# omid-arhami/topolow

Measured on AMD Instinct MI355X. Metric: relaxation iterations/sec (NxN pairs), higher is better.
Workload: dtype f32

## Files before the change

topolow_amd/csrc/relax_kernels.h:

```cpp
#pragma once

#include <hip/hip_runtime.h>
#include <type_traits>
#include "relax_common.h"
#include "relax_prep_types.h"

namespace topolow {

constexpr int kThreads = 256;
constexpr int kWaves = kThreads / 64;

template <int THREADS_, int RPW_, int CHUNK_, int PRIO_ = 0, int MINWAVES_ = 1>
struct StageCfg {
  static constexpr int MINWAVES = MINWAVES_;
  static constexpr int PRIO = PRIO_;
  static constexpr int THREADS = THREADS_;
  static constexpr int WAVES = THREADS_ / 64;
  static constexpr int RPW = RPW_;
  static constexpr int ROWS = WAVES * RPW_;
  static constexpr int CHUNK = CHUNK_;
};

template <typename real> struct Math;
template <> struct Math<float> {
// ... 760 lines not shown
    part_cnt[blockIdx.x] = tc;
  }
}

__global__ __launch_bounds__(1024) void reduce_push_kernel(
    const double* __restrict__ part_sum, const unsigned long long* __restrict__ part_cnt, int n_parts,
    double* const* __restrict__ dst_sum, unsigned long long* const* __restrict__ dst_cnt, int n_dst,
    int slot, const RunState* st) {
  if (st != nullptr && st->stopped) return;
  __shared__ double sh_s[1024];
  __shared__ unsigned long long sh_c[1024];
  double s = 0.0;
  unsigned long long c = 0;
  for (int p = threadIdx.x; p < n_parts; p += 1024) { s += part_sum[p]; c += part_cnt[p]; }
  sh_s[threadIdx.x] = s;
  sh_c[threadIdx.x] = c;
  __syncthreads();
  for (int half = 512; half >= 1; half >>= 1) {
    if (threadIdx.x < half) {
      sh_s[threadIdx.x] += sh_s[threadIdx.x + half];
      sh_c[threadIdx.x] += sh_c[threadIdx.x + half];
    }
    __syncthreads();
  }
  if ((int)threadIdx.x < n_dst) {
    dst_sum[threadIdx.x][slot] = sh_s[0];
    dst_cnt[threadIdx.x][slot] = sh_c[0];
  }
}

__global__ __launch_bounds__(1024) void reduce_total_kernel(
    const double* __restrict__ part_sum, const unsigned long long* __restrict__ part_cnt, int n_parts,
    double* __restrict__ out2, const RunState* st) {
  if (st != nullptr && st->stopped) { if (threadIdx.x == 0) { out2[0] = 0.0; out2[1] = 0.0; } return; }
  __shared__ double sh_s[1024];
  __shared__ unsigned long long sh_c[1024];
  double s = 0.0;
  unsigned long long c = 0;
  for (int p = threadIdx.x; p < n_parts; p += 1024) { s += part_sum[p]; c += part_cnt[p]; }
  sh_s[threadIdx.x] = s;
  sh_c[threadIdx.x] = c;
  __syncthreads();
  for (int half = 512; half >= 1; half >>= 1) {
    if (threadIdx.x < half) {
      sh_s[threadIdx.x] += sh_s[threadIdx.x + half];
      sh_c[threadIdx.x] += sh_c[threadIdx.x + half];
    }
    __syncthreads();
  }
  if (threadIdx.x == 0) { out2[0] = sh_s[0]; out2[1] = (double)sh_c[0]; }
}

constexpr int kCtlThreads = 1024;

template <int THREADS, typename real>
__device__ __forceinline__ void controller_step(
    RunState* st, RunState* mailbox, const double* __restrict__ part_sum,
    const unsigned long long* __restrict__ part_cnt, int n_parts, const real* __restrict__ pos,
    real* __restrict__ best_pos, long long n_values, int iter1, double k_after,
    double* __restrict__ trace, int trace_cap, const double* __restrict__ total2) {
  static_assert(THREADS >= 64 && THREADS <= kCtlThreads && kCtlThreads % THREADS == 0 && (THREADS & (THREADS - 1)) == 0,
                "controller_step: a power-of-two workgroup of at most kCtlThreads threads");
  constexpr int V = kCtlThreads / THREADS;
  if (st->stopped) return;
  __shared__ double sh_s[THREADS];
  __shared__ unsigned long long sh_c[THREADS];
  __shared__ int sh_action;
  double s[V];
  unsigned long long c[V];
#pragma unroll
  for (int j = 0; j < V; ++j) {
    s[j] = 0.0;
    c[j] = 0;
    if (total2 == nullptr)
      for (int p = threadIdx.x + j * THREADS; p < n_parts; p += kCtlThreads) { s[j] += part_sum[p]; c[j] += part_cnt[p]; }
  }
  if (total2 != nullptr && threadIdx.x == 0) { s[0] = total2[0]; c[0] = (unsigned long long)total2[1]; }
#pragma unroll
  for (int h = V / 2; h >= 1; h >>= 1) {
#pragma unroll
    for (int j = 0; j < h; ++j) { s[j] += s[j + h]; c[j] += c[j + h]; }
  }
  sh_s[threadIdx.x] = s[0];
  sh_c[threadIdx.x] = c[0];
  __syncthreads();
  for (int half = THREADS / 2; half >= 1; half >>= 1) {
    if (threadIdx.x < half) {
      sh_s[threadIdx.x] += sh_s[threadIdx.x + half];
      sh_c[threadIdx.x] += sh_c[threadIdx.x + half];
    }
    __syncthreads();
  }
  if (threadIdx.x == 0) {
    const double err = sh_c[0] > 0 ? sh_s[0] / (double)sh_c[0] : 0.0;
    const int action = st->ctl.observe(err, iter1, k_after);
    st->last_mae = err;
    if (trace != nullptr && st->n_checks < trace_cap) {
      trace[3 * st->n_checks + 0] = (double)iter1;
      trace[3 * st->n_checks + 1] = err;
      trace[3 * st->n_checks + 2] = k_after;
    }
    st->n_checks += 1;
    st->iter_base = iter1;
    st->k_base = k_after;
    if (action & 1) { st->stopped = 1; st->converged = 1; }
    sh_action = action;
  }
  __syncthreads();
  if (sh_action & 2) {
    const long long bytes = n_values * (long long)sizeof(real);
    const long long n16 = bytes / 16;
    const uint4* src = reinterpret_cast<const uint4*>(pos);
    uint4* dst = reinterpret_cast<uint4*>(best_pos);
    for (long long q = threadIdx.x; q < n16; q += THREADS) dst[q] = src[q];
    for (long long q = n16 * 16 / (long long)sizeof(real) + threadIdx.x; q < n_values; q += THREADS)
      best_pos[q] = pos[q];
  }
  __syncthreads();
  if (threadIdx.x == 0 && mailbox != nullptr) {
    *mailbox = *st;
    __threadfence_system();
  }
}

template <typename real>
__global__ __launch_bounds__(kCtlThreads) void controller_kernel(
    RunState* st, RunState* mailbox, const double* __restrict__ part_sum,
    const unsigned long long* __restrict__ part_cnt, int n_parts, const real* __restrict__ pos,
    real* __restrict__ best_pos, long long n_values, int iter1, double k_after,
    double* __restrict__ trace, int trace_cap, const double* __restrict__ total2) {
  controller_step<kCtlThreads, real>(st, mailbox, part_sum, part_cnt, n_parts, pos, best_pos, n_values, iter1, k_after,
                                     trace, trace_cap, total2);
}

__global__ __launch_bounds__(kThreads) void encode_dense_kernel(
    const double* __restrict__ D, const int* __restrict__ T, int n, int row_begin, int row_end,
    int ld, uint32_t* __restrict__ out, const int* __restrict__ perm, float* __restrict__ dout) {
  const int c = blockIdx.y * kThreads + threadIdx.x;
  const int i = row_begin + blockIdx.x;
  if (c >= ld || i >= row_end) return;
  uint32_t w = kInfWord;
  float dl = 0.0f;
  if (c < n && c != i) {
    const int oi = perm ? perm[i] : i, oc = perm ? perm[c] : c;
    const int lo = oi < oc ? oi : oc, hi = oi < oc ? oc : oi;
    const size_t cell = (size_t)lo + (size_t)hi * n;
    w = encode_target(D[cell], T[cell]);
    dl = encode_delta(D[cell], w);
  }
  out[enc_index(i - row_begin, c, ld)] = w;
  if (dout != nullptr) dout[enc_index(i - row_begin, c, ld)] = dl;
}


__global__ __launch_bounds__(kPrepThreads) void prep_degree_terms_kernel(const int32_t* __restrict__ degrees, int n,
                                                                          const int* __restrict__ perm,
                                                                          float* __restrict__ gplus) {
  const int q = blockIdx.x * kPrepThreads + threadIdx.x;
  if (q >= n) return;
  gplus[q] = (float)degrees[perm != nullptr ? perm[q] : q] + 1.0f;
}

__global__ __launch_bounds__(kPrepThreads) void prep_session_edges_kernel(
    const int32_t* __restrict__ edge_i, const int32_t* __restrict__ edge_j, const double* __restrict__ edge_dist,
    const int32_t* __restrict__ edge_thresh, long long n_edges, const int* __restrict__ inv, int* __restrict__ ei,
    int* __restrict__ ej, int8_t* __restrict__ ec, double* __restrict__ t64, float* __restrict__ t32) {
  const long long e = (long long)blockIdx.x * kPrepThreads + threadIdx.x;
  if (e >= n_edges) return;
  const int a = edge_i[e], b = edge_j[e];
  ei[e] = inv != nullptr ? inv[a] : a;
  ej[e] = inv != nullptr ? inv[b] : b;
  const int c = edge_thresh[e];
  ec[e] = (int8_t)(c == 0 ? 0 : (c == 1 ? 1 : (c == -1 ? -1 : 2)));
  const double d = edge_dist[e];
  if (t64 != nullptr) t64[e] = d;
  else t32[e] = (float)d;
}

TL_HD inline uint64_t cell_fingerprint(int lo, int hi, uint32_t word) {
  return mix64(((uint64_t)(uint32_t)lo << 32) ^ (uint64_t)(uint32_t)hi ^ ((uint64_t)word * 0x9e3779b97f4a7c15ull));
}
TL_HD inline bool dense_takes(int i, int c, bool parity) {
  if (!parity) return c > i;
  const bool even = ((i + c) & 1) == 0;
  return (even & (c > i)) | (!even & (c < i));
// ... 77 lines not shown
```

topolow_amd/csrc/relax_symm.h:

```cpp
#pragma once

#include <hip/hip_runtime.h>
#include <algorithm>
#include <type_traits>
#include <vector>
#include "relax_common.h"
#include "relax_kernels.h"
#include "relax_symm_plan.h"

namespace topolow {

#ifndef TOPOLOW_SYM_MINW
#define TOPOLOW_SYM_MINW 2
#endif

typedef float symf2 __attribute__((ext_vector_type(2)));
#ifdef TOPOLOW_SYM_STAMPS
__device__ unsigned long long* g_sym_stamps = nullptr;
#endif

#define TL_SYM_DPP_ADD(v, ctrl) asm volatile("v_add_f32_dpp %0, %0, %0 " ctrl " row_mask:0xf bank_mask:0xf" : "+v"(v))
template <int NV>
__device__ __forceinline__ void sym_col_reduce(float (&first)[NV], float (&second)[NV]) {
#pragma unroll
// ... 269 lines not shown
    if constexpr (ERR) {
      double s = (double)err_unit;
#pragma unroll
      for (int m = 32; m >= 1; m >>= 1) s += __shfl_xor(s, m, 64);
      if constexpr (ANYTHR) {
#pragma unroll
        for (int m = 32; m >= 1; m >>= 1) cnt_unit2 += __shfl_xor(cnt_unit2, m, 64);
      }
      if (lane == 0) {
        part_sum[slot] = s;
        part_cnt[slot] = ANYTHR ? (unsigned long long)cnt_unit2 : (slot == 0 ? fixed_cnt : 0ull);
      }
    }
  }
#ifdef TOPOLOW_SYM_STAMPS
  if (lane == 0 && g_sym_stamps != nullptr) {
    g_sym_stamps[4 * gw] = __builtin_amdgcn_s_memtime() - stamp_c0;
    g_sym_stamps[4 * gw + 1] = stamp_r0;
    g_sym_stamps[4 * gw + 2] = __builtin_amdgcn_s_memrealtime();
    unsigned hw_id, xcc_id;
    asm volatile("s_getreg_b32 %0, hwreg(HW_REG_HW_ID)" : "=s"(hw_id));
    asm volatile("s_getreg_b32 %0, hwreg(HW_REG_XCC_ID)" : "=s"(xcc_id));
    g_sym_stamps[4 * gw + 3] = ((unsigned long long)xcc_id << 32) | hw_id;
  }
#endif
}

template <int DIM, typename real> struct SymReal;
template <int DIM> struct SymReal<DIM, float> {
  static constexpr int W = SymRec<DIM>::W;
  __device__ static float ks(double k, float g) { return (float)(2.0 * k) / (4.0f * g + (float)k); }
  __device__ static float cg(double c_rep, float g) { return (float)(0.5 * c_rep) / g; }
  __device__ static float far(int) { return kFarF32; }
};

struct SymApplyCheck {
  const double* part_sum = nullptr;
  const unsigned long long* part_cnt = nullptr;
  int n_parts = 0;
  const void* pos = nullptr;
  void* best = nullptr;
  long long n_values = 0;
  int iter1 = 0;
  double k_after = 0.0;
  double* trace = nullptr;
  int trace_cap = 0;
  RunState* mailbox = nullptr;
};

#ifndef TL_APPLY_PARTS
#define TL_APPLY_PARTS 16
#endif
constexpr int kSymApplyParts = TL_APPLY_PARTS;
template <int DIM, typename real>
__global__ __launch_bounds__(32 * kSymApplyParts) void symm_apply_kernel(
    const real* __restrict__ rec, real* __restrict__ rec_next, real* __restrict__ pos_out, const float* __restrict__ gplus,
    const real* __restrict__ rowpart, const real* __restrict__ colpart, const int2* __restrict__ row_units, int n,
    int npad, double k_next, double c_rep, int iter1, RunState* st, int rr_stages = 0, int rr_stage = 0,
    SymApplyCheck chk = SymApplyCheck{}) {
  const bool check_wg = (int)blockIdx.x * kSymCols >= npad;
  const int R = check_wg ? 0 : blockIdx.x >> 1;
  const int2 ru = row_units[R];
  int stopped = st->stopped;
  asm("" : "+s"(stopped) : "s"(ru.x), "s"(ru.y), "s"(rec), "s"(rowpart), "s"(colpart), "s"(n), "s"(npad), "s"(rr_stages), "s"(rr_stage),
      "s"(rec_next), "s"(pos_out), "s"(gplus), "s"(k_next), "s"(c_rep));
  if (stopped) return;
  if (check_wg) {
    if (chk.part_sum != nullptr)
      controller_step<32 * kSymApplyParts, real>(st, chk.mailbox, chk.part_sum, chk.part_cnt, chk.n_parts,
                                                 (const real*)chk.pos, (real*)chk.best, chk.n_values, chk.iter1,
                                                 chk.k_after, chk.trace, chk.trace_cap, nullptr);
    return;
  }
  using T = SymReal<DIM, real>;
  constexpr int W = T::W;
  constexpr int kWavesA = kSymApplyParts / 2;
  __shared__ real red[kWavesA][kSymCols][DIM];
  const int part = threadIdx.x >> 5, pt = threadIdx.x & 31;
  const int i = blockIdx.x * kSymCols + pt;
  real acc[DIM];
#pragma unroll
  for (int d = 0; d < DIM; ++d) acc[d] = 0;
  int rp0 = 0, rp1 = R;
  if (rr_stages > 0) sym_rr_above(npad / kSymRows, rr_stages, rr_stage, R, rp0, rp1);
  for (int Rp = rp0 + part; Rp < rp1; Rp += kSymApplyParts) {
    const real* src = colpart + ((size_t)Rp * npad + i) * DIM;
#pragma unroll
    for (int d = 0; d < DIM; ++d) acc[d] += src[d];
  }
  const int row_in_tile = i - R * kSymRows;
  for (int q = part; q < ru.y; q += kSymApplyParts) {
    const real* src = rowpart + ((size_t)(ru.x + q) * kSymRows + row_in_tile) * DIM;
#pragma unroll
    for (int d = 0; d < DIM; ++d) acc[d] -= src[d];
  }
#pragma unroll
  for (int d = 0; d < DIM; ++d) {
    if constexpr (std::is_same<real, float>::value) acc[d] += __shfl_xor(acc[d], 32, 64);
    else acc[d] += T::lane_xor(acc[d], 32);
  }
  const int wave = threadIdx.x >> 6;
  if ((threadIdx.x & 32) == 0) {
#pragma unroll
    for (int d = 0; d < DIM; ++d) red[wave][pt][d] = acc[d];
  }
  __syncthreads();
  if (part == 0 && i < n) {
    bool finite = true;
    real out[DIM];
#pragma unroll
    for (int d = 0; d < DIM; ++d) {
      real t = red[0][pt][d];
#pragma unroll
      for (int p = 1; p < kWavesA; ++p) t += red[p][pt][d];
      out[d] = rec[(size_t)i * W + d] + t;
      finite = finite && isfinite(out[d]);
      pos_out[(size_t)i * DIM + d] = out[d];
      rec_next[(size_t)i * W + d] = out[d];
    }
    const real g = (real)gplus[i];
    rec_next[(size_t)i * W + DIM] = T::ks(k_next, g);
    rec_next[(size_t)i * W + DIM + 1] = T::cg(c_rep, g);
    if (!finite) atomicMin(&st->first_nonfinite, iter1);
  }
}

template <int DIM, typename real>
__global__ __launch_bounds__(256) void symm_records_kernel(const real* __restrict__ pos, const float* __restrict__ gplus,
                                                          real* __restrict__ rec, int n, int npad, double k, double c_rep) {
  using T = SymReal<DIM, real>;
  constexpr int W = T::W;
  const int i = blockIdx.x * blockDim.x + threadIdx.x;
  if (i >= npad) return;
  real* r = rec + (size_t)i * W;
  if (i < n) {
#pragma unroll
    for (int d = 0; d < DIM; ++d) r[d] = pos[(size_t)i * DIM + d];
    const real g = (real)gplus[i];
    r[DIM] = T::ks(k, g);
    r[DIM + 1] = T::cg(c_rep, g);
  } else {
#pragma unroll
    for (int d = 0; d < DIM; ++d) r[d] = T::far(d);
    r[DIM] = 0;
    r[DIM + 1] = 0;
  }
#pragma unroll
// ... 107 lines not shown
```

topolow_amd/csrc/topolow_relax.hip:

```cpp

#include "topolow_session.h"
#include "topolow_prep.h"
#include "relax_kernels.h"
#include "relax_exact.h"
#include "relax_tilegs.h"
#include "relax_symm.h"
#include "relax_symm64.h"
#include "relax_symm_wide.h"
#include "relax_cv.h"

namespace {

#define TL_DISPATCH_DIM(dim, FN, ...)                 \
  switch (dim) {                                      \
    case 1: FN<1>(__VA_ARGS__); break;                \
    case 2: FN<2>(__VA_ARGS__); break;                \
    case 3: FN<3>(__VA_ARGS__); break;                \
    case 4: FN<4>(__VA_ARGS__); break;                \
    case 5: FN<5>(__VA_ARGS__); break;                \
    case 6: FN<6>(__VA_ARGS__); break;                \
    case 7: FN<7>(__VA_ARGS__); break;                \
    case 8: FN<8>(__VA_ARGS__); break;                \
    case 9: FN<9>(__VA_ARGS__); break;                \
    case 10: FN<10>(__VA_ARGS__); break;              \
// ... 180 lines not shown
void launch_dense_error(topolow_session* s, const void* pos, const RunState* st) {
  const size_t lds = sizeof(real) * DIM * ErrCfg::CHUNK;
  const dim3 grid(s->dense_grid_x, s->dense_grid_y);
  if (s->dense_parity) {
    hipLaunchKernelGGL((dense_error_kernel<DIM, real, ErrCfg, true>), grid, dim3(ErrCfg::THREADS), lds,
                       s->stream, s->enc.p, s->ld, s->row_begin, s->row_end, s->n, (const real*)pos,
                       s->rowflags.p, s->part_sum.p, s->part_cnt.p, st);
  } else {
    hipLaunchKernelGGL((dense_error_kernel<DIM, real, ErrCfg, false>), grid, dim3(ErrCfg::THREADS), lds,
                       s->stream, s->enc.p, s->ld, s->row_begin, s->row_end, s->n, (const real*)pos,
                       s->rowflags.p, s->part_sum.p, s->part_cnt.p, st);
  }
}

int edge_error_blocks(long long n_edges) {
  long long blocks = (n_edges + (long long)kThreads * 8 - 1) / ((long long)kThreads * 8);
  if (blocks < 1) blocks = 1;
  if (blocks > 2048) blocks = 2048;
  return (int)blocks;
}

int error_parts(const topolow_session* s) { return s->dense_mae ? s->dense_blocks : s->n_parts; }

template <int DIM>
void launch_edge_error(topolow_session* s, const void* pos, const RunState* st) {
  if (s->dense_mae) {
    if constexpr (DIM > kMaxTunedDim) {
      throw HipError{TOPOLOW_ERR_UNSUPPORTED, "dense MAE pass: ndim"};
    } else {
      if (s->precision == TOPOLOW_PRECISION_F64) launch_dense_error<DIM, double>(s, pos, st);
      else launch_dense_error<DIM, float>(s, pos, st);
    }
  } else if (s->precision == TOPOLOW_PRECISION_F64) {
    hipLaunchKernelGGL((edge_error_kernel<DIM, double, double>), dim3(s->n_parts),
                       dim3(kThreads), 0, s->stream, (const double*)pos, s->ei.p, s->ej.p,
                       (const double*)s->et.p, s->ec.p, s->n_edges, s->part_sum.p,
                       s->part_cnt.p, st);
  } else {
    hipLaunchKernelGGL((edge_error_kernel<DIM, float, float>), dim3(s->n_parts), dim3(kThreads),
                       0, s->stream, (const float*)pos, s->ei.p, s->ej.p, (const float*)s->et.p,
                       s->ec.p, s->n_edges, s->part_sum.p, s->part_cnt.p, st);
  }
  HIP_TRY(hipGetLastError());
}

void launch_controller(topolow_session* s, const void* pos, int iter1, double k_after,
                       const double* psum = nullptr, const unsigned long long* pcnt = nullptr, int nparts = 0,
                       const double* total2 = nullptr) {
  const long long nv = (long long)s->n * s->dim;
  if (psum == nullptr && total2 == nullptr) { psum = s->part_sum.p; pcnt = s->part_cnt.p; nparts = error_parts(s); }
  if (s->precision == TOPOLOW_PRECISION_F64) {
    hipLaunchKernelGGL((controller_kernel<double>), dim3(1), dim3(kCtlThreads), 0, s->stream,
                       s->state.p, s->mailbox_dev, psum, pcnt, nparts,
                       (const double*)pos, (double*)s->best.p, nv, iter1, k_after, s->trace_dev, s->trace_cap, total2);
  } else {
    hipLaunchKernelGGL((controller_kernel<float>), dim3(1), dim3(kCtlThreads), 0, s->stream,
                       s->state.p, s->mailbox_dev, psum, pcnt, nparts,
                       (const float*)pos, (float*)s->best.p, nv, iter1, k_after, s->trace_dev, s->trace_cap, total2);
  }
  HIP_TRY(hipGetLastError());
}

void upload_positions(topolow_session* s, const double* host_colmajor, void* dst) {
  const size_t nv = (size_t)s->pos_rows() * s->dim;
  if (s->precision == TOPOLOW_PRECISION_F64) {
    std::vector<double> tmp(nv, 0.0);
    for (int i = 0; i < s->n; ++i) {
      const int o = s->perm.empty() ? i : s->perm[i];
      for (int d = 0; d < s->udim; ++d) tmp[(size_t)i * s->dim + d] = host_colmajor[o + (size_t)d * s->n];
    }
    for (int i = s->n; i < s->pos_rows(); ++i) tmp[(size_t)i * s->dim] = kFarF64;
    HIP_TRY(hipMemcpyAsync(dst, tmp.data(), nv * 8, hipMemcpyHostToDevice, s->stream));
    HIP_TRY(hipStreamSynchronize(s->stream));
  } else {
    std::vector<float> tmp(nv, 0.0f);
    for (int i = 0; i < s->n; ++i) {
      const int o = s->perm.empty() ? i : s->perm[i];
      for (int d = 0; d < s->udim; ++d)
        tmp[(size_t)i * s->dim + d] = (float)host_colmajor[o + (size_t)d * s->n];
    }
    for (int i = s->n; i < s->pos_rows(); ++i) tmp[(size_t)i * s->dim] = kFarF32;
    HIP_TRY(hipMemcpyAsync(dst, tmp.data(), nv * 4, hipMemcpyHostToDevice, s->stream));
    HIP_TRY(hipStreamSynchronize(s->stream));
  }
}

void download_positions(topolow_session* s, const void* src, double* host_colmajor) {
  const size_t nv = (size_t)s->n * s->dim;
  if (s->precision == TOPOLOW_PRECISION_F64) {
    std::vector<double> tmp(nv);
    HIP_TRY(hipMemcpyAsync(tmp.data(), src, nv * 8, hipMemcpyDeviceToHost, s->stream));
    HIP_TRY(hipStreamSynchronize(s->stream));
    for (int i = 0; i < s->n; ++i) {
      const int o = s->perm.empty() ? i : s->perm[i];
      for (int d = 0; d < s->udim; ++d) host_colmajor[o + (size_t)d * s->n] = tmp[(size_t)i * s->dim + d];
    }
  } else {
    std::vector<float> tmp(nv);
    HIP_TRY(hipMemcpyAsync(tmp.data(), src, nv * 4, hipMemcpyDeviceToHost, s->stream));
    HIP_TRY(hipStreamSynchronize(s->stream));
    for (int i = 0; i < s->n; ++i) {
      const int o = s->perm.empty() ? i : s->perm[i];
      for (int d = 0; d < s->udim; ++d)
        host_colmajor[o + (size_t)d * s->n] = (double)tmp[(size_t)i * s->dim + d];
    }
  }
}

void scan_row_flags(topolow_session* s) {
  DevBuf<unsigned long long> measured;
  measured.alloc(1);
// ... 274 lines not shown
}

template <int DIM>
void sym_sweep(topolow_session* s, const SymPlanDev& plan, const void* rec, bool thr, bool err,
               unsigned long long block_cells, int col_row0, bool prio) {
  auto& y = s->sym;
  if (err && ((size_t)plan.n_units > s->part_sum.n || (size_t)plan.n_units > s->part_cnt.n))
    throw HipError{TOPOLOW_ERR_HIP, "symmetric sweep: the error partials are smaller than the plan's unit count"};
  sym_real<DIM>(s, [&](auto r) {
    using real = decltype(r);
    sym_sweep_instance<DIM, real>(thr, err, s->exact, [&](auto kern) {
      if constexpr (std::is_same<real, double>::value)
        hipLaunchKernelGGL(kern, dim3(y.grid), dim3(64 * kSymWaves), 0, s->stream, y.tenc.p, (const double*)rec,
                           plan.units.p, plan.runs.p, (double*)y.rowpart.p, (double*)y.colpart.p, y.npad, s->state.p,
                           col_row0, y.tdelta.p, s->part_sum.p, s->part_cnt.p, block_cells);
      else
        hipLaunchKernelGGL(kern, dim3(y.grid), dim3(64 * kSymWaves), 0, s->stream, y.tenc.p, (const float*)rec,
                           plan.units.p, plan.runs.p, (float*)y.rowpart.p, (float*)y.colpart.p, y.npad, s->state.p,
                           s->part_sum.p, s->part_cnt.p, block_cells, col_row0, prio && y.prio ? 1 : 0);
    });
  });
}

bool sym_fused_ok(const topolow_session* s) {
  if (!s->sym.delta_ready) return false;
  return !s->exact || (s->list_is_block && s->n_edges > 0 && s->sym.holds == SymHolds::kTriangle);
}

template <int DIM>
void sym_apply(topolow_session* s, const SymPlanDev& plan, const void* rec, void* rec_next, void* pout, double k_next,
               int iter, int rr_stages, int rr_stage, const PendingCheck* chk = nullptr, const void* pin = nullptr,
               int n_parts = 0) {
  auto& y = s->sym;
  SymApplyCheck ac;
  if (chk != nullptr) {
    ac.part_sum = s->part_sum.p;
    ac.part_cnt = s->part_cnt.p;
    ac.n_parts = n_parts;
    ac.pos = pin;
    ac.best = s->best.p;
    ac.n_values = (long long)s->n * s->dim;
    ac.iter1 = chk->iter1;
    ac.k_after = chk->k_after;
    ac.trace = s->trace_dev;
    ac.trace_cap = s->trace_cap;
    ac.mailbox = s->mailbox_dev;
  }
  sym_real<DIM>(s, [&](auto r) {
    using real = decltype(r);
    hipLaunchKernelGGL((symm_apply_kernel<DIM, real>), dim3(y.npad / kSymCols + (chk != nullptr ? 1 : 0)),
                       dim3(32 * kSymApplyParts), 0, s->stream,
                       (const real*)rec, (real*)rec_next, (real*)pout, s->gplus.p, (const real*)y.rowpart.p,
                       (const real*)y.colpart.p, plan.row_units.p, s->n, y.npad, k_next, s->c_rep, iter + 1, s->state.p,
                       rr_stages, rr_stage, ac);
  });
}

bool sym_rr_stages_ok(int S) { return S == 2 || S == 4 || S == 8; }
int sym_rr_log2(int S) { return S == 2 ? 1 : (S == 4 ? 2 : 3); }

SymPlan sym_rr_plan(int npad, int n_waves, int S, int st) {
  const int TR = npad / kSymRows;
  return relax_symm_plan_rows(npad, n_waves, [&](int R, int& j0, int& j1) { sym_rr_row(TR, S, st, R, j0, j1); });
}

bool sym_rr_available(topolow_session* s, int S) {
  auto& y = s->sym;
  if (!sym_rr_stages_ok(S) || y.holds != SymHolds::kTriangle) return false;
  const int TR = y.npad / kSymRows;
  if (TR < 2 * S) return false;
  if ((long long)TR * (TR + 1) / S < (long long)y.rr_min_tiles * y.grid * kSymWaves) return false;
  const int lg = sym_rr_log2(S);
  if (!y.rr[lg].empty()) return true;
  std::vector<SymPlanDev> plans(S);
  for (int st = 0; st < S; ++st) {
    const SymPlan hp = sym_rr_plan(y.npad, y.grid * kSymWaves, S, st);
    if (hp.units.size() * kSymRows * s->dim * s->real_size() > y.rowpart.n) return false;
    plans[st].load(hp);
  }
  y.rr[lg] = std::move(plans);
  return true;
}

template <int DIM>
void sym_iteration(topolow_session* s, const void* pin, void* pout, int iter, double k, bool err, int S = 0, int st = 0,
                   bool last = true, const PendingCheck* in_apply = nullptr) {
  auto& y = s->sym;
  const SymPlanDev& plan = S == 0 ? y.plan : y.rr[sym_rr_log2(S)][st];
  ProfScope prof(s, S > 0 ? &s->prof_stage : err ? &s->prof_sym_err : &s->prof_sym);
  if (err && s->precision == TOPOLOW_PRECISION_F64 && !sym_fused_ok(s))
    throw HipError{TOPOLOW_ERR_UNSUPPORTED, "symmetric sweep (f64): no delta tiles for a fused check"};
  if (y.rec_iter != iter) {
    for (int b = 0; b < 2; ++b)
      sym_records<DIM>(s, pin, y.rec[b].p, k);
    y.rec_cur = 0;
  }
  sym_sweep<DIM>(s, plan, y.rec[y.rec_cur].p, s->any_threshold, err, S == 0 ? s->block_cells : 0ull, 0, true);
  if (in_apply != nullptr && !(err && S == 0))
    throw HipError{TOPOLOW_ERR_BAD_ARGUMENT, "symmetric sweep: a check in the apply needs the ERR sweep of a one-stage iteration"};
  sym_apply<DIM>(s, plan, y.rec[y.rec_cur].p, y.rec[y.rec_cur ^ 1].p, pout, last ? k * (1.0 - s->cooling) : k, iter, S, st,
                 in_apply, pin, plan.n_units);
  HIP_TRY(hipGetLastError());
  y.rec_cur ^= 1;
  y.rec_iter = last ? iter + 1 : iter;
  if (err) s->fused_parts = plan.n_units;
  s->stage_launches += 1;
}
// ... 700 lines not shown
  }
  if (row_begin < 0 || row_end > n || row_begin >= row_end) {
    set_err(errbuf, errlen, "bad row block [%d,%d) for n=%d", row_begin, row_end, n);
    return TOPOLOW_ERR_BAD_ARGUMENT;
  }
  const bool exact = precision == TOPOLOW_PRECISION_F64_EXACT;
  if (exact && (row_begin != 0 || row_end != n)) {
    set_err(errbuf, errlen, "precision f64_exact: whole-problem sessions only (rows [%d,%d) of %d asked for): the row-sharded "
            "paths have no exact kernels", row_begin, row_end, n);
    return TOPOLOW_ERR_UNSUPPORTED;
  }
  if (exact && ndim > kMaxTunedDim) {
    set_err(errbuf, errlen, "precision f64_exact: ndim must be between 1 and %d (the plain stage kernel of wider embeddings "
            "reads the 4-byte targets only)", kMaxTunedDim);
    return TOPOLOW_ERR_UNSUPPORTED;
  }
  topolow_session* s = nullptr;
  const int rc = guarded(errbuf, errlen, [&] {
    const int dev = select_device(device);
    s = new topolow_session();
    s->device = dev;
    s->n = n;
    s->dim = kernel_dim(ndim);
    s->udim = ndim;
    s->row_begin = row_begin;
    s->row_end = row_end;
    s->ld = (n + kEncLdAlign - 1) & ~(kEncLdAlign - 1);
    s->precision = precision == TOPOLOW_PRECISION_F64 || exact ? TOPOLOW_PRECISION_F64 : TOPOLOW_PRECISION_F32;
    s->exact = exact;
    HIP_TRY(hipStreamCreateWithFlags(&s->own_stream, hipStreamNonBlocking));
    s->stream = s->own_stream;
    HIP_TRY(hipStreamCreateWithFlags(&s->check_stream, hipStreamNonBlocking));
    HIP_TRY(hipEventCreateWithFlags(&s->ev_iter_done, hipEventDisableTiming));
    HIP_TRY(hipEventCreateWithFlags(&s->ev_check_done, hipEventDisableTiming));
    const char* serial = getenv("TOPOLOW_SERIAL_CHECKS");
    s->serial_checks = serial != nullptr && serial[0] == '1';
    const char* fuse = getenv("TOPOLOW_FUSE_CHECKS");
    s->fuse_checks = !(fuse != nullptr && fuse[0] == '0');
    const char* in_apply = getenv("TOPOLOW_CHECK_IN_APPLY");
    s->check_in_apply = !(in_apply != nullptr && in_apply[0] == '0');
    const char* symm = getenv("TOPOLOW_SYMMETRIC");
    s->sym.allowed = !(symm != nullptr && symm[0] == '0');
    s->sym.forced = symm != nullptr && symm[0] == '1';
    const char* symm_min = getenv("TOPOLOW_SYMMETRIC_MIN_N");
    s->sym.min_n = symm_min != nullptr ? atoi(symm_min) : kSymMinPoints;
    const char* symm2 = getenv("TOPOLOW_SYMMETRIC_TWO_STAGE");
    s->sym.two_stage = !(symm2 != nullptr && symm2[0] == '0');
    const char* rr_min = getenv("TOPOLOW_SYMMETRIC_STAGE_MIN_TILES");
    if (rr_min != nullptr) s->sym.rr_min_tiles = std::max(0, atoi(rr_min));
    const char* sym_grid = getenv("TOPOLOW_SYMMETRIC_GRID");
    s->sym.grid_cap = sym_grid != nullptr ? std::max(0, atoi(sym_grid)) : 0;
    const char* sym_prio = getenv("TOPOLOW_SYM_PRIO");
    s->sym.prio = !(sym_prio != nullptr && sym_prio[0] == '0');
    s->enc.alloc((size_t)((s->rows() + kEncRowAlign - 1) / kEncRowAlign * kEncRowAlign) * s->ld);
    if (s->exact) s->denc.alloc(s->enc.n);
    const size_t pos_bytes = (size_t)s->pos_rows() * s->dim * s->real_size();
    for (auto& b : s->pos) b.alloc(pos_bytes);
    s->best.alloc(pos_bytes);
    s->state.alloc(1);
    HIP_TRY(hipHostMalloc((void**)&s->mailbox, sizeof(RunState), hipHostMallocMapped));
    std::memset(s->mailbox, 0, sizeof(RunState));
    HIP_TRY(hipHostGetDevicePointer((void**)&s->mailbox_dev, s->mailbox, 0));
  });
  if (rc != TOPOLOW_OK) { delete s; return rc; }
  *out = s;
  return TOPOLOW_OK;
}

void topolow_session_destroy(topolow_session* s) {
  if (!s) return;
  (void)hipSetDevice(s->device);
  if (s->stream) (void)hipStreamSynchronize(s->stream);
  if (s->check_stream) (void)hipStreamSynchronize(s->check_stream);
#ifdef TOPOLOW_TUNING
  g_stamps.dump();
#endif
  delete s;
}

int topolow_session_set_relabel(topolow_session* s, uint64_t seed, char* errbuf, size_t errlen) {
  if (!s) return TOPOLOW_ERR_BAD_ARGUMENT;
  if (s->gplus.p || s->part_sum.p) {
    set_err(errbuf, errlen, "the relabelling must be chosen before targets, edges or positions are loaded");
    return TOPOLOW_ERR_BAD_ARGUMENT;
  }
  return guarded(errbuf, errlen, [&] {
    HIP_TRY(hipSetDevice(s->device));
    s->perm.clear();
    s->inv.clear();
    if (seed == 0) return;
    const int n = s->n;
    s->perm.resize(n);
    s->inv.resize(n);
    for (int q = 0; q < n; ++q) s->perm[q] = q;
    for (int q = n - 1; q > 0; --q) {
      const uint32_t r = rnd_below(rnd64(seed, 0x7e1abe1ull, (uint64_t)q), (uint32_t)(q + 1));
      std::swap(s->perm[q], s->perm[r]);
    }
    for (int q = 0; q < n; ++q) s->inv[s->perm[q]] = q;
    s->d_perm.alloc(n);
    s->d_inv.alloc(n);
    HIP_TRY(hipMemcpy(s->d_perm.p, s->perm.data(), sizeof(int) * (size_t)n, hipMemcpyHostToDevice));
    HIP_TRY(hipMemcpy(s->d_inv.p, s->inv.data(), sizeof(int) * (size_t)n, hipMemcpyHostToDevice));
  });
}

// ... 1070 lines not shown
```

topolow_amd/csrc/topolow_session.h:

```cpp
#pragma once

#include <hip/hip_runtime.h>

#include <chrono>
#include <cstdarg>
#include <cstdio>
#include <algorithm>
#include <cstring>
#include <cstdlib>
#include <array>
#include <atomic>
#include <deque>
#include <functional>
#include <future>
#include <limits>
#include <mutex>
#include <string>
#include <memory>
#include <thread>
#include <vector>

#include "../../include/topolow_relax.h"
#include "relax_common.h"
#include "relax_host.h"
// ... 115 lines not shown
  bool began = false;
  bool in_run = false;
  long long stage_launches = 0;
  std::deque<hipEvent_t> pending;
  std::vector<hipEvent_t> event_pool;
  DevBuf<void*> push_tab[3];
  int n_push = 0;
  DevBuf<double> rank_sum;
  DevBuf<unsigned long long> rank_cnt;
  DevBuf<double*> rsum_tab;
  DevBuf<unsigned long long*> rcnt_tab;
  int n_ranks = 0, rank = 0;
  struct SymState {
    bool allowed = false;
    bool forced = false;
    int min_n = 0;
    enum class Holds {
      kNothing,
      kTriangle,
      kRunSegment,
      kCallerSegment,
    };
    Holds holds = Holds::kNothing;
    int npad = 0, tiles = 0, grid = 0;
    DevBuf<uint32_t> tenc;
    DevBuf<unsigned char> rec[2], rowpart, colpart;
    int rec_cur = 0, rec_iter = -1;
    DevBuf<float> tdelta;
    bool delta_ready = false;
    int generation = 0;
    struct Plan {
      DevBuf<SymUnit> units;
      DevBuf<SymRun> runs;
      DevBuf<int2> row_units;
      int n_units = 0;
      void load(const SymPlan& hp) {
        const std::vector<SymRun> hr = hp.runs();
        n_units = (int)hp.units.size();
        units.alloc(std::max<size_t>(hp.units.size(), 1));
        runs.alloc(hr.size());
        row_units.alloc(std::max<size_t>(hp.row_units.size(), 1));
        if (!hp.units.empty())
          HIP_TRY(hipMemcpy(units.p, hp.units.data(), hp.units.size() * sizeof(SymUnit), hipMemcpyHostToDevice));
        HIP_TRY(hipMemcpy(runs.p, hr.data(), hr.size() * sizeof(SymRun), hipMemcpyHostToDevice));
        if (!hp.row_units.empty())
          HIP_TRY(hipMemcpy(row_units.p, hp.row_units.data(), hp.row_units.size() * sizeof(int2), hipMemcpyHostToDevice));
      }
      void release() { units.release(); runs.release(); row_units.release(); n_units = 0; }
    };
    Plan plan;
    std::vector<Plan> rr[4];
    bool two_stage = true;
    bool prio = true;
    int rr_min_tiles = 5;
    int grid_cap = 0;
    DevBuf<const uint32_t*> src_tab;
    DevBuf<int> src_row0;
    bool seg_thr = false;
    int seg_first = 0, seg_last = -1;
    int seg_slots = 0;
    int seg_slot = 0;
    DevBuf<float> inbox;
    DevBuf<float*> inbox_tab;
    DevBuf<int> own0;
    using Sources = std::vector<std::pair<const void*, unsigned long long>>;
    Sources seg_from;

    void hold(Holds what) { holds = what; }
    void invalidate() {
      holds = Holds::kNothing;
      delta_ready = false;
      rec_iter = -1;
      seg_from.clear();
    }
    void release() {
      tenc.release(); rec[0].release(); rec[1].release(); rowpart.release(); colpart.release();
      tdelta.release();
      plan.release();
      for (auto& v : rr) v.clear();
      src_tab.release(); src_row0.release();
      inbox.release(); inbox_tab.release(); own0.release();
      invalidate();
    }
  } sym;
  struct CvHold {
    bool active = false;
    long long n_pairs = 0;
    DevBuf<int> lo, hi;
    DevBuf<uint32_t> words;
    DevBuf<float> deltas;
    bool tiles_patched = false;
    int generation = 0;
    bool list_compacted = false;
    DevBuf<int> ei, ej;
    DevBuf<unsigned char> et;
    DevBuf<int8_t> ec;
    long long full_edges = 0;
    int full_parts = 0;
    DevBuf<int> blk_count;
    DevBuf<long long> blk_offset;
    DevBuf<int> sc_i, sc_j;
    DevBuf<double> sc_t, sc_part;
  } cv;
  int fused_parts = 0;
  bool profiling = false;
  std::vector<std::pair<hipEvent_t, hipEvent_t>> prof_stage, prof_stage_err, prof_check;
// ... 30 lines not shown
```

Measured before the change: 18840.

## Batch partial-sum loads with buffer intrinsics in symm apply and controller

Rewrites the symmetric apply kernel's column and row partial accumulation to issue several bounds-checked raw buffer loads per wave before reducing, with waves striding over pairs of strips. The controller's partial-sum reduction and best-position snapshot copy get the same batching. The goal is more memory-level parallelism and less per-iteration latency in these small reduction loops. A TOPOLOW_APPLY_BATCH env switch controls it. The cost is more register pressure and more complex indexing that relies on buffer out-of-range loads returning zero.

```diff
diff --git a/topolow_amd/csrc/relax_kernels.h b/topolow_amd/csrc/relax_kernels.h
--- a/topolow_amd/csrc/relax_kernels.h
+++ b/topolow_amd/csrc/relax_kernels.h
@@ -836,13 +836,15 @@
 }
 
 constexpr int kCtlThreads = 1024;
+constexpr int kCtlBatch = 4;
+constexpr int kCtlSnapBatch = 8;
 
 template <int THREADS, typename real>
 __device__ __forceinline__ void controller_step(
     RunState* st, RunState* mailbox, const double* __restrict__ part_sum,
     const unsigned long long* __restrict__ part_cnt, int n_parts, const real* __restrict__ pos,
     real* __restrict__ best_pos, long long n_values, int iter1, double k_after,
-    double* __restrict__ trace, int trace_cap, const double* __restrict__ total2) {
+    double* __restrict__ trace, int trace_cap, const double* __restrict__ total2, int snap_batch) {
   static_assert(THREADS >= 64 && THREADS <= kCtlThreads && kCtlThreads % THREADS == 0 && (THREADS & (THREADS - 1)) == 0,
                 "controller_step: a power-of-two workgroup of at most kCtlThreads threads");
   constexpr int V = kCtlThreads / THREADS;
@@ -856,8 +858,33 @@
   for (int j = 0; j < V; ++j) {
     s[j] = 0.0;
     c[j] = 0;
-    if (total2 == nullptr)
-      for (int p = threadIdx.x + j * THREADS; p < n_parts; p += kCtlThreads) { s[j] += part_sum[p]; c[j] += part_cnt[p]; }
+  }
+  if (total2 == nullptr) {
+    typedef unsigned int u32x2 __attribute__((ext_vector_type(2)));
+    const __amdgpu_buffer_rsrc_t sum_rsrc =
+        __builtin_amdgcn_make_buffer_rsrc(const_cast<double*>(part_sum), 0, n_parts * 8, 0x00020000);
+    const __amdgpu_buffer_rsrc_t cnt_rsrc =
+        __builtin_amdgcn_make_buffer_rsrc(const_cast<unsigned long long*>(part_cnt), 0, n_parts * 8, 0x00020000);
+    for (int base = 0; base < n_parts; base += kCtlBatch * kCtlThreads) {
+      u32x2 ws[V][kCtlBatch], wc[V][kCtlBatch];
+#pragma unroll
+      for (int j = 0; j < V; ++j)
+#pragma unroll
+        for (int k = 0; k < kCtlBatch; ++k) {
+          const int p = base + k * kCtlThreads + j * THREADS + (int)threadIdx.x;
+          ws[j][k] = __builtin_amdgcn_raw_buffer_load_b64(sum_rsrc, p * 8, 0, 0);
+          wc[j][k] = __builtin_amdgcn_raw_buffer_load_b64(cnt_rsrc, p * 8, 0, 0);
+        }
+      __builtin_amdgcn_sched_barrier(0);
+#pragma unroll
+      for (int j = 0; j < V; ++j)
+#pragma unroll
+        for (int k = 0; k < kCtlBatch; ++k)
+          if (base + k * kCtlThreads + j * THREADS + (int)threadIdx.x < n_parts) {
+            s[j] += __builtin_bit_cast(double, ws[j][k]);
+            c[j] += __builtin_bit_cast(unsigned long long, wc[j][k]);
+          }
+    }
   }
   if (total2 != nullptr && threadIdx.x == 0) { s[0] = total2[0]; c[0] = (unsigned long long)total2[1]; }
 #pragma unroll
@@ -891,14 +918,29 @@
     sh_action = action;
   }
   __syncthreads();
-  if (sh_action & 2) {
+  if (__builtin_amdgcn_readfirstlane(sh_action) & 2) {
+    typedef unsigned int u32x4 __attribute__((ext_vector_type(4)));
     const long long bytes = n_values * (long long)sizeof(real);
     const long long n16 = bytes / 16;
     const uint4* src = reinterpret_cast<const uint4*>(pos);
     uint4* dst = reinterpret_cast<uint4*>(best_pos);
-    for (long long q = threadIdx.x; q < n16; q += THREADS) dst[q] = src[q];
-    for (long long q = n16 * 16 / (long long)sizeof(real) + threadIdx.x; q < n_values; q += THREADS)
-      best_pos[q] = pos[q];
+    const int trip = (snap_batch ? kCtlSnapBatch : 1) * THREADS;
+    for (long long q0 = 0; q0 < n16; q0 += trip) {
+      const int pieces = n16 - q0 < trip ? (int)(n16 - q0) : trip;
+      const __amdgpu_buffer_rsrc_t src_rsrc =
+          __builtin_amdgcn_make_buffer_rsrc(const_cast<uint4*>(src + q0), 0, pieces * 16, 0x00020000);
+      const __amdgpu_buffer_rsrc_t dst_rsrc = __builtin_amdgcn_make_buffer_rsrc(dst + q0, 0, pieces * 16, 0x00020000);
+      u32x4 v[kCtlSnapBatch];
+#pragma unroll
+      for (int j = 0; j < kCtlSnapBatch; ++j)
+        v[j] = __builtin_amdgcn_raw_buffer_load_b128(src_rsrc, (j * THREADS + (int)threadIdx.x) * 16, 0, 0);
+      __builtin_amdgcn_sched_barrier(0);
+#pragma unroll
+      for (int j = 0; j < kCtlSnapBatch; ++j)
+        __builtin_amdgcn_raw_buffer_store_b128(v[j], dst_rsrc, (j * THREADS + (int)threadIdx.x) * 16, 0, 0);
+    }
+    const long long q = n16 * 16 / (long long)sizeof(real) + threadIdx.x;
+    if (q < n_values) best_pos[q] = pos[q];
   }
   __syncthreads();
   if (threadIdx.x == 0 && mailbox != nullptr) {
@@ -912,9 +954,9 @@
     RunState* st, RunState* mailbox, const double* __restrict__ part_sum,
     const unsigned long long* __restrict__ part_cnt, int n_parts, const real* __restrict__ pos,
     real* __restrict__ best_pos, long long n_values, int iter1, double k_after,
-    double* __restrict__ trace, int trace_cap, const double* __restrict__ total2) {
+    double* __restrict__ trace, int trace_cap, const double* __restrict__ total2, int snap_batch) {
   controller_step<kCtlThreads, real>(st, mailbox, part_sum, part_cnt, n_parts, pos, best_pos, n_values, iter1, k_after,
-                                     trace, trace_cap, total2);
+                                     trace, trace_cap, total2, snap_batch);
 }
 
 __global__ __launch_bounds__(kThreads) void encode_dense_kernel(
diff --git a/topolow_amd/csrc/relax_symm.h b/topolow_amd/csrc/relax_symm.h
--- a/topolow_amd/csrc/relax_symm.h
+++ b/topolow_amd/csrc/relax_symm.h
@@ -345,12 +345,41 @@
 #define TL_APPLY_PARTS 16
 #endif
 constexpr int kSymApplyParts = TL_APPLY_PARTS;
+constexpr int kSymApplyBatch = 4;
+
+template <int NW>
+__device__ __forceinline__ void sym_strip_request(__amdgpu_buffer_rsrc_t rsrc, int byte_off, uint32_t (&w)[NW]) {
+  typedef unsigned int u32x2 __attribute__((ext_vector_type(2)));
+  typedef unsigned int u32x3 __attribute__((ext_vector_type(3)));
+  typedef unsigned int u32x4 __attribute__((ext_vector_type(4)));
+  constexpr int kFull = NW / 4, kRest = NW % 4;
+#pragma unroll
+  for (int v = 0; v < kFull; ++v) {
+    const u32x4 q = __builtin_amdgcn_raw_buffer_load_b128(rsrc, byte_off + 16 * v, 0, 0);
+    w[4 * v + 0] = q.x; w[4 * v + 1] = q.y; w[4 * v + 2] = q.z; w[4 * v + 3] = q.w;
+  }
+  if constexpr (kRest == 3) {
+    const u32x3 q = __builtin_amdgcn_raw_buffer_load_b96(rsrc, byte_off + 16 * kFull, 0, 0);
+    w[4 * kFull + 0] = q.x; w[4 * kFull + 1] = q.y; w[4 * kFull + 2] = q.z;
+  } else if constexpr (kRest == 2) {
+    const u32x2 q = __builtin_amdgcn_raw_buffer_load_b64(rsrc, byte_off + 16 * kFull, 0, 0);
+    w[4 * kFull + 0] = q.x; w[4 * kFull + 1] = q.y;
+  } else if constexpr (kRest == 1) {
+    w[4 * kFull] = __builtin_amdgcn_raw_buffer_load_b32(rsrc, byte_off + 16 * kFull, 0, 0);
+  }
+}
+template <typename real, int NW>
+__device__ __forceinline__ real sym_strip_value(const uint32_t (&w)[NW], int d) {
+  if constexpr (sizeof(real) == 4) return __builtin_bit_cast(float, w[d]);
+  else return __builtin_bit_cast(double, ((unsigned long long)w[2 * d + 1] << 32) | w[2 * d]);
+}
+
 template <int DIM, typename real>
 __global__ __launch_bounds__(32 * kSymApplyParts) void symm_apply_kernel(
     const real* __restrict__ rec, real* __restrict__ rec_next, real* __restrict__ pos_out, const float* __restrict__ gplus,
     const real* __restrict__ rowpart, const real* __restrict__ colpart, const int2* __restrict__ row_units, int n,
     int npad, double k_next, double c_rep, int iter1, RunState* st, int rr_stages = 0, int rr_stage = 0,
-    SymApplyCheck chk = SymApplyCheck{}) {
+    SymApplyCheck chk = SymApplyCheck{}, int batch = 1) {
   const bool check_wg = (int)blockIdx.x * kSymCols >= npad;
   const int R = check_wg ? 0 : blockIdx.x >> 1;
   const int2 ru = row_units[R];
@@ -362,7 +391,7 @@
     if (chk.part_sum != nullptr)
       controller_step<32 * kSymApplyParts, real>(st, chk.mailbox, chk.part_sum, chk.part_cnt, chk.n_parts,
                                                  (const real*)chk.pos, (real*)chk.best, chk.n_values, chk.iter1,
-                                                 chk.k_after, chk.trace, chk.trace_cap, nullptr);
+                                                 chk.k_after, chk.trace, chk.trace_cap, nullptr, batch);
     return;
   }
   using T = SymReal<DIM, real>;
@@ -376,16 +405,55 @@
   for (int d = 0; d < DIM; ++d) acc[d] = 0;
   int rp0 = 0, rp1 = R;
   if (rr_stages > 0) sym_rr_above(npad / kSymRows, rr_stages, rr_stage, R, rp0, rp1);
-  for (int Rp = rp0 + part; Rp < rp1; Rp += kSymApplyParts) {
-    const real* src = colpart + ((size_t)Rp * npad + i) * DIM;
-#pragma unroll
-    for (int d = 0; d < DIM; ++d) acc[d] += src[d];
-  }
+  constexpr int NW = DIM * (int)sizeof(real) / 4;
+  const int wave2 = 2 * __builtin_amdgcn_readfirstlane((int)threadIdx.x >> 6);
+  const int odd = part & 1;
+  const int bw = batch ? kSymApplyBatch : 1;
+  const int col_bytes = npad * DIM * (int)sizeof(real);
+  constexpr int kUnitBytes = kSymRows * DIM * (int)sizeof(real);
   const int row_in_tile = i - R * kSymRows;
-  for (int q = part; q < ru.y; q += kSymApplyParts) {
-    const real* src = rowpart + ((size_t)(ru.x + q) * kSymRows + row_in_tile) * DIM;
-#pragma unroll
-    for (int d = 0; d < DIM; ++d) acc[d] -= src[d];
+  const int col_off = odd * col_bytes + i * DIM * (int)sizeof(real);
+  const int row_off = (odd * kSymRows + row_in_tile) * DIM * (int)sizeof(real);
+  auto col_rsrc = [&](int Rw, int j) {
+    const int rows = j >= bw ? 0 : std::min(std::max(rp1 - Rw, 0), 2);
+    const unsigned long long at = ((unsigned long long)__umulhi((unsigned)Rw, (unsigned)col_bytes) << 32) | ((unsigned)Rw * (unsigned)col_bytes);
+    return __builtin_amdgcn_make_buffer_rsrc(reinterpret_cast<char*>(const_cast<real*>(colpart)) + at, 0, __builtin_amdgcn_readfirstlane(rows * col_bytes), 0x00020000);
+  };
+  auto row_rsrc = [&](int qw, int j) {
+    const int units = j >= bw ? 0 : std::min(std::max(ru.y - qw, 0), 2);
+    return __builtin_amdgcn_make_buffer_rsrc(const_cast<real*>(rowpart) + (size_t)(ru.x + qw) * kSymRows * DIM, 0, __builtin_amdgcn_readfirstlane(units * kUnitBytes), 0x00020000);
+  };
+  uint32_t rw[kSymApplyBatch][NW], cw[kSymApplyBatch][NW];
+#pragma unroll
+  for (int j = 0; j < kSymApplyBatch; ++j)
+    sym_strip_request<NW>(row_rsrc(wave2 + j * kSymApplyParts, j), row_off, rw[j]);
+  for (int Rw = rp0 + wave2; Rw < rp1; Rw += bw * kSymApplyParts) {
+#pragma unroll
+    for (int j = 0; j < kSymApplyBatch; ++j)
+      sym_strip_request<NW>(col_rsrc(Rw + j * kSymApplyParts, j), col_off, cw[j]);
+    __builtin_amdgcn_sched_barrier(0);
+#pragma unroll
+    for (int j = 0; j < kSymApplyBatch; ++j) {
+      const bool on = j < bw && Rw + j * kSymApplyParts + odd < rp1;
+#pragma unroll
+      for (int d = 0; d < DIM; ++d) acc[d] = on ? acc[d] + sym_strip_value<real>(cw[j], d) : acc[d];
+    }
+  }
+  auto subtract_rows = [&](int qw) {
+#pragma unroll
+    for (int j = 0; j < kSymApplyBatch; ++j) {
+      const bool on = j < bw && qw + j * kSymApplyParts + odd < ru.y;
+#pragma unroll
+      for (int d = 0; d < DIM; ++d) acc[d] = on ? acc[d] - sym_strip_value<real>(rw[j], d) : acc[d];
+    }
+  };
+  subtract_rows(wave2);
+  for (int qw = wave2 + bw * kSymApplyParts; qw < ru.y; qw += bw * kSymApplyParts) {
+#pragma unroll
+    for (int j = 0; j < kSymApplyBatch; ++j)
+      sym_strip_request<NW>(row_rsrc(qw + j * kSymApplyParts, j), row_off, rw[j]);
+    __builtin_amdgcn_sched_barrier(0);
+    subtract_rows(qw);
   }
 #pragma unroll
   for (int d = 0; d < DIM; ++d) {
diff --git a/topolow_amd/csrc/topolow_relax.hip b/topolow_amd/csrc/topolow_relax.hip
--- a/topolow_amd/csrc/topolow_relax.hip
+++ b/topolow_amd/csrc/topolow_relax.hip
@@ -256,11 +256,13 @@
   if (s->precision == TOPOLOW_PRECISION_F64) {
     hipLaunchKernelGGL((controller_kernel<double>), dim3(1), dim3(kCtlThreads), 0, s->stream,
                        s->state.p, s->mailbox_dev, psum, pcnt, nparts,
-                       (const double*)pos, (double*)s->best.p, nv, iter1, k_after, s->trace_dev, s->trace_cap, total2);
+                       (const double*)pos, (double*)s->best.p, nv, iter1, k_after, s->trace_dev, s->trace_cap, total2,
+                       s->sym.apply_batch ? 1 : 0);
   } else {
     hipLaunchKernelGGL((controller_kernel<float>), dim3(1), dim3(kCtlThreads), 0, s->stream,
                        s->state.p, s->mailbox_dev, psum, pcnt, nparts,
-                       (const float*)pos, (float*)s->best.p, nv, iter1, k_after, s->trace_dev, s->trace_cap, total2);
+                       (const float*)pos, (float*)s->best.p, nv, iter1, k_after, s->trace_dev, s->trace_cap, total2,
+                       s->sym.apply_batch ? 1 : 0);
   }
   HIP_TRY(hipGetLastError());
 }
@@ -641,7 +643,7 @@
                        dim3(32 * kSymApplyParts), 0, s->stream,
                        (const real*)rec, (real*)rec_next, (real*)pout, s->gplus.p, (const real*)y.rowpart.p,
                        (const real*)y.colpart.p, plan.row_units.p, s->n, y.npad, k_next, s->c_rep, iter + 1, s->state.p,
-                       rr_stages, rr_stage, ac);
+                       rr_stages, rr_stage, ac, y.apply_batch ? 1 : 0);
   });
 }
 
@@ -1448,6 +1450,8 @@
     s->sym.grid_cap = sym_grid != nullptr ? std::max(0, atoi(sym_grid)) : 0;
     const char* sym_prio = getenv("TOPOLOW_SYM_PRIO");
     s->sym.prio = !(sym_prio != nullptr && sym_prio[0] == '0');
+    const char* apply_batch = getenv("TOPOLOW_APPLY_BATCH");
+    s->sym.apply_batch = !(apply_batch != nullptr && apply_batch[0] == '0');
     s->enc.alloc((size_t)((s->rows() + kEncRowAlign - 1) / kEncRowAlign * kEncRowAlign) * s->ld);
     if (s->exact) s->denc.alloc(s->enc.n);
     const size_t pos_bytes = (size_t)s->pos_rows() * s->dim * s->real_size();
diff --git a/topolow_amd/csrc/topolow_session.h b/topolow_amd/csrc/topolow_session.h
--- a/topolow_amd/csrc/topolow_session.h
+++ b/topolow_amd/csrc/topolow_session.h
@@ -191,6 +191,7 @@
     std::vector<Plan> rr[4];
     bool two_stage = true;
     bool prio = true;
+    bool apply_batch = true;
     int rr_min_tiles = 5;
     int grid_cap = 0;
     DevBuf<const uint32_t*> src_tab;
```

New measurement: 18840, median of 2. Within noise of the previous version (-0.0%).
